# Golbstein/Keras-segmentation-deeplab-v3.1

Hardware: AMD Instinct MI355X
Metric: images/sec fwd+bwd, 512x512 MobileNetV2 OS=16, 21 classes (higher is better)
Workload: dtype f32; 1 GPU; Deeplabv3(backbone='mobilenetv2', input_shape=(512,512,3), classes=21, OS=16) head=deeplab: fwd + sparse-xent loss + bwd + Adam, BN batch mode, dropout 0.1; global_batch=128, per_gpu_batch=128, parallelism=dp1, hipgraph=True, matrix_math=f32, dist_strict=False, backward_fork=False

## Files before the change

keras-segmentation-deeplab-v3.1_amd/csrc/pwws.hip:

```cpp
#include "common.h"
#include "pwargs.h"
namespace {
using pw::GemmArgs;

template <int KQ, int TN, int OC>
__global__ __launch_bounds__(256, OC) void pw_fwd_ws_kernel(GemmArgs P) {
  constexpr int KH = 4 * KQ, K = 8 * KQ, NP = 32 * TN;
  __shared__ float Ws[K * NP];
  __shared__ float cf[2 * K];
  __shared__ float bs[NP];
  __shared__ float Cs[4 * 1024];
  static_assert(sizeof(float) * (K * NP + 2 * K + NP + 4 * 1024) * OC <= 160 * 1024, "weight-stationary kernel: OC workgroups do not fit a gfx950 CU's LDS");
  const int tid = threadIdx.x, lane = tid & 63;
  const int wave = __builtin_amdgcn_readfirstlane(tid >> 6);
  const int l31 = lane & 31, lhi = lane >> 5;
  const bool xform = (P.ka != nullptr);

  for (int i = tid; i < K * NP; i += 256) {
    const int k = i / NP, n = i % NP;
    Ws[i] = n < P.N ? P.b[(size_t)k * P.ldb + n] : 0.f;
  }
  for (int i = tid; i < K; i += 256) {
    cf[i] = xform ? P.ka[i] : 1.f;
    cf[K + i] = xform ? P.kc[i] : 0.f;
  }
  for (int i = tid; i < NP; i += 256) bs[i] = (P.bias && i < P.N) ? P.bias[i] : 0.f;
  float st1[TN], st2[TN];
#pragma unroll
  for (int j = 0; j < TN; j++) st1[j] = st2[j] = 0.f;
  __syncthreads();

  const int nfull = P.M >> 5;
  const int gw = blockIdx.x * 4 + wave, GW = gridDim.x * 4;
  float *const cw = Cs + wave * 1024;
  const float *const wfrag = Ws + KH * lhi * NP + l31;
  const float *const cfs = cf + KH * lhi, *const cft = cf + K + KH * lhi;
  const int c4 = (lane & 7) * 4, r0 = lane >> 3;
  const int c4l = c4 % (P.N - 32 * (TN - 1));

  f32x4 nx[KQ];
  auto load_tile = [&](int t) {
    const int row = min(t * 32 + l31, P.M - 1);
    const float *p = P.a + (size_t)row * P.lda + KH * lhi;
#pragma unroll
    for (int j = 0; j < KQ; j++) nx[j] = ld4(p + 4 * j);
  };
  auto mfma_tile = [&](f32x16 (&acc)[TN], int next) {
#pragma unroll
    for (int q = 0; q < KQ; q++) {
      const f32x4 v = dl3_act4(ld4(cfs + 4 * q) * nx[q] + ld4(cft + 4 * q), P.a_act);
#pragma unroll
      for (int e = 0; e < 4; e++)
#pragma unroll
        for (int j = 0; j < TN; j++)
          acc[j] = __builtin_amdgcn_mfma_f32_32x32x2f32(v[e], wfrag[(4 * q + e) * NP + j * 32], acc[j], 0, 0, 0);
    }
    __builtin_amdgcn_sched_barrier(0);
    if (next >= 0) load_tile(next);
    __builtin_amdgcn_sched_barrier(0);
  };

  if (gw < nfull) load_tile(gw);
  __builtin_amdgcn_s_waitcnt(0x0F70);
  for (int t = gw; t < nfull; t += GW) {
    f32x16 acc[TN];
#pragma unroll
    for (int j = 0; j < TN; j++)
#pragma unroll
      for (int r = 0; r < 16; r++) acc[j][r] = 0.f;
    mfma_tile(acc, t + GW < nfull ? t + GW : -1);
    float *const cp = P.c + (size_t)(t * 32 + r0) * P.ldc;
#pragma unroll
    for (int j = 0; j < TN; j++) {
      const float bj = bs[j * 32 + l31];
#pragma unroll
      for (int r = 0; r < 16; r++) {
        const float v = acc[j][r] + bj;
        st1[j] += v;
        st2[j] += v * v;
        cw[((r & 3) + 8 * (r >> 2) + 4 * lhi) * 32 + l31] = v;
      }
      __builtin_amdgcn_wave_barrier();
      const int cc = (j == TN - 1) ? c4l : c4;
      f32x4 o[4];
#pragma unroll
      for (int p = 0; p < 4; p++) o[p] = ld4(cw + (r0 + 8 * p) * 32 + cc);
#pragma unroll
      for (int p = 0; p < 4; p++) st4_nt(cp + (size_t)(8 * p) * P.ldc + j * 32 + cc, o[p]);
      __builtin_amdgcn_wave_barrier();
    }
  }
  if ((P.M & 31) != 0 && gw == nfull % GW) {
    f32x16 acc[TN];
#pragma unroll
    for (int j = 0; j < TN; j++)
#pragma unroll
      for (int r = 0; r < 16; r++) acc[j][r] = 0.f;
    load_tile(nfull);
    mfma_tile(acc, -1);
    const int m0 = nfull * 32;
#pragma unroll
    for (int j = 0; j < TN; j++) {
      const int col = j * 32 + l31;
      const float bj = bs[col];
#pragma unroll
      for (int r = 0; r < 16; r++) {
        const int row = m0 + (r & 3) + 8 * (r >> 2) + 4 * lhi;
        const float v = acc[j][r] + bj;
        if (row < P.M && col < P.N) {
          st1[j] += v;
          st2[j] += v * v;
          P.c[(size_t)row * P.ldc + col] = v;
        }
      }
    }
  }

  if (P.stat_mode != 0) {
    __syncthreads();
    float *sred = Cs;
#pragma unroll
    for (int j = 0; j < TN; j++) {
      const float a1 = st1[j] + __shfl_xor(st1[j], 32, 64), a2 = st2[j] + __shfl_xor(st2[j], 32, 64);
      if (lhi == 0) {
        sred[(wave * NP + j * 32 + l31) * 2 + 0] = a1;
        sred[(wave * NP + j * 32 + l31) * 2 + 1] = a2;
      }
    }
    __syncthreads();
    for (int cl = tid; cl < NP; cl += 256) {
      if (cl < P.N) {
        float a1 = 0.f, a2 = 0.f;
#pragma unroll
        for (int w = 0; w < 4; w++) {
          a1 += sred[(w * NP + cl) * 2 + 0];
          a2 += sred[(w * NP + cl) * 2 + 1];
        }
        P.part[((size_t)blockIdx.x * P.N + cl) * 2 + 0] = a1;
        P.part[((size_t)blockIdx.x * P.N + cl) * 2 + 1] = a2;
        for (int r = blockIdx.x + (int)gridDim.x; r < P.part_rows; r += (int)gridDim.x) {
          P.part[((size_t)r * P.N + cl) * 2 + 0] = 0.f;
          P.part[((size_t)r * P.N + cl) * 2 + 1] = 0.f;
        }
      }
    }
  }
}

#ifndef DL3_WS2_XPRE_TN
#define DL3_WS2_XPRE_TN 4
#endif
template <int KQ, int TN, int NW, bool BWD = false, bool TWO = false, bool ADD = false, bool FLAT = false>
__global__ __launch_bounds__(64 * NW) void pw_ws2_kernel(GemmArgs P) {
  static_assert(BWD || (!TWO && !ADD), "two-tensor operand / residual addend: bwd-data only");
  static_assert(!FLAT || (!BWD && TN == 1), "packed narrow output: forward, one column block");
  constexpr bool XPRE = BWD && !TWO && TN <= DL3_WS2_XPRE_TN;
  constexpr int KH = 4 * KQ, K = 8 * KQ, NP = 32 * TN;
  __shared__ __attribute__((aligned(16))) float Ws[K * NP];
  __shared__ __attribute__((aligned(16))) float cf[(TWO ? 3 : 2) * K];
  __shared__ __attribute__((aligned(16))) float bs[BWD ? 4 * NP : NP];
  __shared__ __attribute__((aligned(16))) float Cs[NW * 1024];
  static_assert(sizeof(float) * (K * NP + 3 * K + 4 * NP + NW * 1024) <= 160 * 1024, "gfx950: 160 KB of LDS per CU");
  const int tid = threadIdx.x, lane = tid & 63;
  const int wave = __builtin_amdgcn_readfirstlane(tid >> 6);
  const int l31 = lane & 31, lhi = lane >> 5;
  const int nwg = gridDim.x * gridDim.y, b = blockIdx.y * gridDim.x + blockIdx.x;
  const int xq = nwg >> 3, xr = nwg & 7, xcd = b & 7;
  const int lid = (xcd < xr ? xcd * (xq + 1) : xr * (xq + 1) + (xcd - xr) * xq) + (b >> 3);
  const int ct = lid % gridDim.x, rg = lid / gridDim.x, nrg = gridDim.y;
  const int n0 = ct * NP;
  const bool xform = (P.ka != nullptr);

  for (int i = tid; i < K * NP; i += 64 * NW) {
    const int k = i / NP, n = n0 + i % NP;
    Ws[i] = n < P.N ? P.b[(size_t)k * P.ldb + n] : 0.f;
  }
  for (int i = tid; i < K; i += 64 * NW) {
    cf[i] = xform ? P.ka[i] : 1.f;
    cf[K + i] = xform ? P.kc[i] : 0.f;
    if constexpr (TWO) cf[2 * K + i] = P.kb[i];
  }
  for (int i = tid; i < NP; i += 64 * NW) {
    const int col = min(n0 + i, P.N - 1);
    if constexpr (BWD) {
      bs[i] = P.ep_scale ? P.ep_scale[col] : 1.f;
      bs[NP + i] = P.ep_scale ? P.ep_shift[col] : 0.f;
      bs[2 * NP + i] = P.stat_mode == 2 ? P.ep_mean[col] : 0.f;
      bs[3 * NP + i] = P.stat_mode == 2 ? P.ep_invstd[col] : 0.f;
    } else {
      bs[i] = (P.bias && n0 + i < P.N) ? P.bias[n0 + i] : 0.f;
    }
  }
  float st1[TN], st2[TN];
#pragma unroll
  for (int j = 0; j < TN; j++) st1[j] = st2[j] = 0.f;
  f32x4 q1[BWD ? TN : 1], q2[BWD ? TN : 1];
  if constexpr (BWD) {
#pragma unroll
    for (int j = 0; j < TN; j++) q1[j] = q2[j] = splat4(0.f);
  }
  __syncthreads();

  const int nfull = P.M >> 5;
  const int gw = rg * NW + wave, GW = nrg * NW;
  float *const cw = Cs + wave * 1024;
  const float *const wfrag = Ws + KH * lhi * NP + l31;
  const float *const cfs = cf + KH * lhi, *const cft = cf + K + KH * lhi;
  const int c4 = (lane & 7) * 4, r0 = lane >> 3;
  const int ncol = min(NP, P.N - n0);
  const int jl = (ncol - 1) >> 5;
  const int c4l = FLAT ? 0 : c4 % (ncol - 32 * jl);

  constexpr int NCH = BWD ? KQ / 2 : 4;
  static_assert(NCH % 2 == 0, "an even number of chunks per tile");
  constexpr int SQ = KQ / NCH;
  static_assert(KQ % NCH == 0, "the reduction must split into an even number of equal chunks");
  f32x4 nx[2][SQ], ny[2][TWO ? SQ : 1];
  auto req = [&](int t, int c, int sl) __attribute__((always_inline)) {
    const int row = min(t * 32 + l31, P.M - 1);
    const float *p = P.a + (size_t)row * P.lda + KH * lhi + 4 * SQ * c;
#pragma unroll
    for (int j = 0; j < SQ; j++) nx[sl][j] = ld4(p + 4 * j);
    if constexpr (TWO) {
      const float *p2 = P.a2 + (size_t)row * P.lda2 + KH * lhi + 4 * SQ * c;
#pragma unroll
      for (int j = 0; j < SQ; j++) ny[sl][j] = ld4(p2 + 4 * j);
    }
  };
  auto mfma_tile = [&](f32x16 (&acc)[TN], int t, int tn) __attribute__((always_inline)) {
    float bf[2][TN];
#pragma unroll
    for (int j = 0; j < TN; j++) bf[0][j] = wfrag[j * 32];
#pragma unroll
    for (int c = 0; c < NCH; c++) {
#pragma unroll
      for (int q = 0; q < SQ; q++) {
        const int kq = SQ * c + q;
        f32x4 v;
        if constexpr (TWO) {
          v = ld4(cfs + 4 * kq) * nx[c & 1][q] + ld4(cft + 4 * kq);
          v += ld4(cf + 2 * K + KH * lhi + 4 * kq) * ny[c & 1][q];
        } else if constexpr (BWD) {
          v = nx[c & 1][q];
        } else {
          v = dl3_act4(ld4(cfs + 4 * kq) * nx[c & 1][q] + ld4(cft + 4 * kq), P.a_act);
        }
#pragma unroll
        for (int e = 0; e < 4; e++) {
          const int ks = 4 * kq + e, cur = ks & 1;
          if (ks + 1 < KH) {
#pragma unroll
            for (int j = 0; j < TN; j++) bf[cur ^ 1][j] = wfrag[(ks + 1) * NP + j * 32];
          }
#pragma unroll
          for (int j = 0; j < TN; j++) acc[j] = __builtin_amdgcn_mfma_f32_32x32x2f32(v[e], bf[cur][j], acc[j], 0, 0, 0);
          __builtin_amdgcn_sched_group_barrier(0x100, TN, 0);
          __builtin_amdgcn_sched_group_barrier(0x008, TN, 0);
        }
      }
      __builtin_amdgcn_sched_barrier(0);
      if (c + 2 < NCH) req(t, c + 2, c & 1);
      else req(tn, c + 2 - NCH, c & 1);
      __builtin_amdgcn_sched_barrier(0);
    }
  };

  if (gw < nfull) {
    req(gw, 0, 0);
    req(gw, 1, 1);
  }
  __builtin_amdgcn_s_waitcnt(0x0F70);
  for (int t = gw; t < nfull; t += GW) {
    f32x16 acc[TN];
#pragma unroll
    for (int j = 0; j < TN; j++)
#pragma unroll
      for (int r = 0; r < 16; r++) acc[j][r] = 0.f;
    f32x4 xq[BWD ? 2 : 1][BWD ? 4 : 1], aq[BWD ? 2 : 1][ADD ? 4 : 1];
    if constexpr (XPRE) {
      int le = lane, c4le = c4l;
      asm volatile("" : "+v"(le), "+v"(c4le));
      const int c4 = (le & 7) * 4, r0 = le >> 3, c4l = c4le;
      const float *const xp0 = P.ep_x + (size_t)(t * 32 + r0) * P.ld_epx + n0;
      const float *const ap0 = ADD ? P.ep_add + (size_t)(t * 32 + r0) * P.ld_add + n0 : nullptr;
#pragma unroll
      for (int jj = 0; jj < (TN < 2 ? TN : 2); jj++) {
        const int cc_ = jj < jl ? jj * 32 + c4 : jl * 32 + c4l;
#pragma unroll
        for (int p = 0; p < 4; p++) {
          xq[jj][p] = ld4(xp0 + (size_t)(8 * p) * P.ld_epx + cc_);
          if constexpr (ADD) aq[jj][p] = ld4(ap0 + (size_t)(8 * p) * P.ld_add + cc_);
        }
      }
    }
    mfma_tile(acc, t, t + GW < nfull ? t + GW : t);
    if constexpr (BWD) {
      int le = lane, c4le = c4l;
      asm volatile("" : "+v"(le), "+v"(c4le));
      const int c4 = (le & 7) * 4, r0 = le >> 3, l31 = le & 31, lhi = le >> 5, c4l = c4le;
      float *const cp = P.c + (size_t)(t * 32 + r0) * P.ldc + n0;
      const float *const xp = P.ep_x + (size_t)(t * 32 + r0) * P.ld_epx + n0;
      const float *const ap = ADD ? P.ep_add + (size_t)(t * 32 + r0) * P.ld_add + n0 : nullptr;
      if constexpr (!XPRE) {
#pragma unroll
        for (int p = 0; p < 4; p++) {
          xq[0][p] = ld4(xp + (size_t)(8 * p) * P.ld_epx + (0 == jl ? c4l : c4));
          if constexpr (ADD) aq[0][p] = ld4(ap + (size_t)(8 * p) * P.ld_add + (0 == jl ? c4l : c4));
        }
      }
#pragma unroll
      for (int j = 0; j < TN; j++) {
        if (j <= jl) {
          if (!XPRE && j + 1 <= jl) {
#pragma unroll
            for (int p = 0; p < 4; p++) {
              xq[(j + 1) & 1][p] = ld4(xp + (size_t)(8 * p) * P.ld_epx + (j + 1) * 32 + (j + 1 == jl ? c4l : c4));
              if constexpr (ADD) aq[(j + 1) & 1][p] = ld4(ap + (size_t)(8 * p) * P.ld_add + (j + 1) * 32 + (j + 1 == jl ? c4l : c4));
            }
          }
#pragma unroll
          for (int r = 0; r < 16; r++) cw[((r & 3) + 8 * (r >> 2) + 4 * lhi) * 32 + l31] = acc[j][r];
          __builtin_amdgcn_wave_barrier();
          const int cc = (j == jl) ? c4l : c4;
          const f32x4 es = ld4(bs + j * 32 + cc), et = ld4(bs + NP + j * 32 + cc);
          const f32x4 mu = ld4(bs + 2 * NP + j * 32 + cc), is = ld4(bs + 3 * NP + j * 32 + cc);
          const float own = (cc == c4) ? 1.f : 0.f;
#pragma unroll
          for (int p = 0; p < 4; p++) {
            const f32x4 x = xq[j & 1][p];
            f32x4 o = ld4(cw + (r0 + 8 * p) * 32 + cc) * dl3_mask4(es * x + et, P.ep_act);
            if constexpr (ADD) o += P.add_scale * aq[j & 1][p];
            st4_nt(cp + (size_t)(8 * p) * P.ldc + j * 32 + cc, o);
            q1[j] += own * o;
            q2[j] += own * (o * ((x - mu) * is));
          }
          if (XPRE && j + 2 <= jl) {
            __builtin_amdgcn_sched_barrier(0);
#pragma unroll
            for (int p = 0; p < 4; p++) {
              xq[j & 1][p] = ld4(xp + (size_t)(8 * p) * P.ld_epx + (j + 2) * 32 + (j + 2 == jl ? c4l : c4));
              if constexpr (ADD) aq[j & 1][p] = ld4(ap + (size_t)(8 * p) * P.ld_add + (j + 2) * 32 + (j + 2 == jl ? c4l : c4));
            }
          }
          __builtin_amdgcn_wave_barrier();
        }
      }
    } else if constexpr (FLAT) {
      const float bj = bs[l31];
      float *const cq = cw + 4 * lhi * P.N + l31;
#pragma unroll
      for (int r = 0; r < 16; r++) {
        const float v = acc[0][r] + bj;
        st1[0] += v;
        st2[0] += v * v;
        if (l31 < P.N) cq[((r & 3) + 8 * (r >> 2)) * P.N] = v;
      }
      __builtin_amdgcn_wave_barrier();
      float *const cp = P.c + (size_t)t * 32 * P.N;
#pragma unroll
      for (int p = 0; p < 4; p++) {
        const int piece = lane + 64 * p;
        if (piece < 8 * P.N) st4_nt(cp + 4 * piece, ld4(cw + 4 * piece));
      }
      __builtin_amdgcn_wave_barrier();
    } else {
    float *const cp = P.c + (size_t)(t * 32 + r0) * P.ldc + n0;
#pragma unroll
    for (int j = 0; j < TN; j++) {
      if (j <= jl) {
        const float bj = bs[j * 32 + l31];
#pragma unroll
        for (int r = 0; r < 16; r++) {
          const float v = acc[j][r] + bj;
          st1[j] += v;
          st2[j] += v * v;
          cw[((r & 3) + 8 * (r >> 2) + 4 * lhi) * 32 + l31] = v;
        }
        __builtin_amdgcn_wave_barrier();
        const int cc = (j == jl) ? c4l : c4;
        f32x4 o[4];
#pragma unroll
        for (int p = 0; p < 4; p++) o[p] = ld4(cw + (r0 + 8 * p) * 32 + cc);
#pragma unroll
        for (int p = 0; p < 4; p++) st4_nt(cp + (size_t)(8 * p) * P.ldc + j * 32 + cc, o[p]);
        __builtin_amdgcn_wave_barrier();
      }
    }
    }
  }
  if ((P.M & 31) != 0 && gw == nfull % GW) {
    f32x16 acc[TN];
#pragma unroll
    for (int j = 0; j < TN; j++)
#pragma unroll
      for (int r = 0; r < 16; r++) acc[j][r] = 0.f;
    __builtin_amdgcn_s_waitcnt(0x0F70);
    req(nfull, 0, 0);
    req(nfull, 1, 1);
    mfma_tile(acc, nfull, nfull);
    const int m0 = nfull * 32;
#pragma unroll
    for (int j = 0; j < TN; j++) {
      const int col = n0 + j * 32 + l31;
      const float bj = BWD ? 0.f : bs[j * 32 + l31];
#pragma unroll
      for (int r = 0; r < 16; r++) {
        const int row = m0 + (r & 3) + 8 * (r >> 2) + 4 * lhi;
        float v = acc[j][r] + bj;
        if (row < P.M && col < P.N) {
          if constexpr (BWD) {
            const float x = P.ep_x[(size_t)row * P.ld_epx + col];
            v *= dl3_act_mask(bs[j * 32 + l31] * x + bs[NP + j * 32 + l31], P.ep_act);
            if constexpr (ADD) v += P.add_scale * P.ep_add[(size_t)row * P.ld_add + col];
            st1[j] += v;
            st2[j] += v * ((x - bs[2 * NP + j * 32 + l31]) * bs[3 * NP + j * 32 + l31]);
          } else {
            st1[j] += v;
            st2[j] += v * v;
          }
          P.c[(size_t)row * P.ldc + col] = v;
        }
      }
    }
  }

  if (P.stat_mode != 0) {
    __syncthreads();
    float *sred = Cs;
    if constexpr (BWD) {
#pragma unroll
      for (int j = 0; j < TN; j++) {
#pragma unroll
        for (int o = 8; o <= 32; o <<= 1) {
#pragma unroll
          for (int e = 0; e < 4; e++) {
            q1[j][e] += __shfl_xor(q1[j][e], o, 64);
            q2[j][e] += __shfl_xor(q2[j][e], o, 64);
          }
        }
        if (lane < 8) {
#pragma unroll
          for (int e = 0; e < 4; e++) {
            sred[(wave * NP + j * 32 + c4 + e) * 2 + 0] = q1[j][e];
            sred[(wave * NP + j * 32 + c4 + e) * 2 + 1] = q2[j][e];
          }
        }
      }
      __builtin_amdgcn_wave_barrier();
    }
#pragma unroll
    for (int j = 0; j < TN; j++) {
      const float a1 = st1[j] + __shfl_xor(st1[j], 32, 64), a2 = st2[j] + __shfl_xor(st2[j], 32, 64);
      if (lhi == 0) {
        sred[(wave * NP + j * 32 + l31) * 2 + 0] = (BWD ? sred[(wave * NP + j * 32 + l31) * 2 + 0] : 0.f) + a1;
        sred[(wave * NP + j * 32 + l31) * 2 + 1] = (BWD ? sred[(wave * NP + j * 32 + l31) * 2 + 1] : 0.f) + a2;
      }
    }
    __syncthreads();
    for (int cl = tid; cl < NP; cl += 64 * NW) {
      const int col = n0 + cl;
      if (col < P.N) {
        float a1 = 0.f, a2 = 0.f;
#pragma unroll
        for (int w = 0; w < NW; w++) {
          a1 += sred[(w * NP + cl) * 2 + 0];
          a2 += sred[(w * NP + cl) * 2 + 1];
        }
        P.part[((size_t)rg * P.N + col) * 2 + 0] = a1;
        P.part[((size_t)rg * P.N + col) * 2 + 1] = a2;
        for (int r = rg + nrg; r < P.part_rows; r += nrg) {
          P.part[((size_t)r * P.N + col) * 2 + 0] = 0.f;
          P.part[((size_t)r * P.N + col) * 2 + 1] = 0.f;
        }
      }
    }
  }
}

template <int TN, int NW>
__global__ __launch_bounds__(64 * NW) void pw_narrowk_kernel(GemmArgs P) {
  constexpr int NP = 32 * TN;
  __shared__ __attribute__((aligned(16))) float Bs[32 * NP];
  __shared__ __attribute__((aligned(16))) float As[NW * 1024];
  __shared__ __attribute__((aligned(16))) float Cs[NW * 1024];
  static_assert(sizeof(float) * (32 * NP + 2 * NW * 1024) <= 160 * 1024, "gfx950: 160 KB of LDS per CU");
  const int tid = threadIdx.x, lane = tid & 63;
  const int wave = __builtin_amdgcn_readfirstlane(tid >> 6);
  const int l31 = lane & 31, lhi = lane >> 5;
  const int n0 = blockIdx.y * NP;
  for (int i = tid; i < 32 * NP; i += 64 * NW) {
    const int k = i / NP, n = n0 + i % NP;
    Bs[i] = (k < P.K && n < P.N) ? P.b[(size_t)k * P.ldb + n] : 0.f;
  }
  __syncthreads();
  const int KS = (P.K + 1) >> 1;
  const int npc = 8 * P.K;
  const int nfull = P.M >> 5;
  const int gw = blockIdx.x * NW + wave, GW = gridDim.x * NW;
  float *const as = As + wave * 1024, *const cw = Cs + wave * 1024;
  const int c4 = (lane & 7) * 4, r0 = lane >> 3;
  f32x4 f[4];
  auto req = [&](int t) __attribute__((always_inline)) {
    const float *p = P.a + (size_t)t * 32 * P.K;
#pragma unroll
    for (int q = 0; q < 4; q++)
      if (lane + 64 * q < npc) f[q] = ld4(p + 4 * (lane + 64 * q));
  };
  auto products = [&](f32x16 (&acc)[TN]) __attribute__((always_inline)) {
#pragma unroll
    for (int j = 0; j < TN; j++)
#pragma unroll
      for (int r = 0; r < 16; r++) acc[j][r] = 0.f;
    const float *ap = as + l31 * P.K + lhi * KS;
    const float *bp = Bs + lhi * KS * NP + l31;
    for (int s = 0; s < KS; s++) {
      const float a = (lhi * KS + s < P.K) ? ap[s] : 0.f;
#pragma unroll
      for (int j = 0; j < TN; j++) acc[j] = __builtin_amdgcn_mfma_f32_32x32x2f32(a, bp[s * NP + j * 32], acc[j], 0, 0, 0);
    }
  };
  if (gw < nfull) req(gw);
  for (int t = gw; t < nfull; t += GW) {
#pragma unroll
    for (int q = 0; q < 4; q++)
      if (lane + 64 * q < npc) st4(as + 4 * (lane + 64 * q), f[q]);
    __builtin_amdgcn_wave_barrier();
    req(t + GW < nfull ? t + GW : t);
    f32x16 acc[TN];
    products(acc);
    float *const cp = P.c + (size_t)(t * 32 + r0) * P.ldc + n0 + c4;
#pragma unroll
    for (int j = 0; j < TN; j++) {
      if (n0 + j * 32 < P.N) {
#pragma unroll
        for (int r = 0; r < 16; r++) cw[((r & 3) + 8 * (r >> 2) + 4 * lhi) * 32 + l31] = acc[j][r];
        __builtin_amdgcn_wave_barrier();
        f32x4 o[4];
#pragma unroll
        for (int p = 0; p < 4; p++) o[p] = ld4(cw + (r0 + 8 * p) * 32 + c4);
#pragma unroll
        for (int p = 0; p < 4; p++) st4_nt(cp + (size_t)(8 * p) * P.ldc + j * 32, o[p]);
        __builtin_amdgcn_wave_barrier();
      }
    }
  }
  if ((P.M & 31) != 0 && gw == nfull % GW) {
    const int m0 = nfull * 32;
    const size_t total = (size_t)P.M * P.K;
    for (int i = lane; i < 32 * P.K; i += 64) {
      const size_t e = (size_t)m0 * P.K + i;
      as[i] = e < total ? P.a[e] : 0.f;
    }
    __builtin_amdgcn_wave_barrier();
    f32x16 acc[TN];
    products(acc);
#pragma unroll
    for (int j = 0; j < TN; j++) {
      const int col = n0 + j * 32 + l31;
#pragma unroll
      for (int r = 0; r < 16; r++) {
        const int row = m0 + (r & 3) + 8 * (r >> 2) + 4 * lhi;
        if (row < P.M && col < P.N) P.c[(size_t)row * P.ldc + col] = acc[j][r];
      }
    }
  }
}
}

void pw::launch_ws(const GemmArgs &A, const GemmPlan &P, void *stream) {
  constexpr int NW = DL3_WS2_NW;
  const dim3 grid(P.grid[0], P.grid[1], P.grid[2]), blk(256), blkw(64 * NW);
#define DL3_GO(KERNEL_, BLK_) hipLaunchKernelGGL((KERNEL_), grid, BLK_, P.lds, (hipStream_t)stream, A)
  switch (P.kernel) {
    case PW_NARROW_FLAT: DL3_GO((pw_ws2_kernel<32, 1, NW, false, false, false, true>), blkw); break;
    case PW_NARROWK: DL3_GO((pw_narrowk_kernel<8, NW>), blkw); break;
    case PW_WS2:
      if (P.two) {
        if (P.add) DL3_GO((pw_ws2_kernel<48, 2, NW, true, true, true>), blkw);
        else DL3_GO((pw_ws2_kernel<48, 2, NW, true, true, false>), blkw);
      } else if (!P.fwd) {
        switch (P.tn) {
          case 5: DL3_GO((pw_ws2_kernel<20, 5, NW, true>), blkw); break;
          case 3: DL3_GO((pw_ws2_kernel<12, 3, NW, true>), blkw); break;
          default: DL3_GO((pw_ws2_kernel<8, 4, NW, true>), blkw); break;
        }
      } else {
        switch (P.tn) {
          case 5: DL3_GO((pw_ws2_kernel<20, 5, NW>), blkw); break;
          case 3: DL3_GO((pw_ws2_kernel<12, 3, NW>), blkw); break;
          default: DL3_GO((pw_ws2_kernel<8, 4, NW>), blkw); break;
        }
      }
      break;
    default:
      switch (P.kq * 10 + P.tn) {
        case 23: DL3_GO((pw_fwd_ws_kernel<2, 3, 4>), blk); break;
        case 35: DL3_GO((pw_fwd_ws_kernel<3, 5, 3>), blk); break;
        case 41: DL3_GO((pw_fwd_ws_kernel<4, 1, 4>), blk); break;
        case 46: DL3_GO((pw_fwd_ws_kernel<4, 6, 3>), blk); break;
        case 121: DL3_GO((pw_fwd_ws_kernel<12, 1, 4>), blk); break;
        case 181: DL3_GO((pw_fwd_ws_kernel<18, 1, 3>), blk); break;
        default: DL3_GO((pw_fwd_ws_kernel<24, 1, 3>), blk); break;
      }
  }
#undef DL3_GO
}
```

Measured before the change: 1345 img/s.

## Load A tiles as coalesced row lines and transpose through LDS in ws2 GEMM

Adds an alternative A-operand path in the weight-stationary pointwise GEMM. Each wave loads contiguous 16-float segments of 8 rows per instruction, applies the BN/activation transform, writes the result to a swizzled per-wave LDS scratch, and reads it back in MFMA fragment order. This replaces the per-lane strided row loads and is meant to improve global-memory coalescing for KQ==8 and two-tensor variants. The cost is extra LDS traffic and wave barriers on every chunk, plus more register use for the staging buffers.

```diff
diff --git a/keras-segmentation-deeplab-v3.1_amd/csrc/pwws.hip b/keras-segmentation-deeplab-v3.1_amd/csrc/pwws.hip
--- a/keras-segmentation-deeplab-v3.1_amd/csrc/pwws.hip
+++ b/keras-segmentation-deeplab-v3.1_amd/csrc/pwws.hip
@@ -149,6 +149,9 @@
 
 #ifndef DL3_WS2_XPRE_TN
 #define DL3_WS2_XPRE_TN 4
+#endif
+#ifndef DL3_WS2_LINES
+#define DL3_WS2_LINES 7
 #endif
 template <int KQ, int TN, int NW, bool BWD = false, bool TWO = false, bool ADD = false, bool FLAT = false>
 __global__ __launch_bounds__(64 * NW) void pw_ws2_kernel(GemmArgs P) {
@@ -211,6 +214,7 @@
   const int jl = (ncol - 1) >> 5;
   const int c4l = FLAT ? 0 : c4 % (ncol - 32 * jl);
 
+  constexpr bool LINES = (TWO && (DL3_WS2_LINES & 1)) || (KQ == 8 && BWD && !TWO && (DL3_WS2_LINES & 2)) || (KQ == 8 && !BWD && (DL3_WS2_LINES & 4));
   constexpr int NCH = BWD ? KQ / 2 : 4;
   static_assert(NCH % 2 == 0, "an even number of chunks per tile");
   constexpr int SQ = KQ / NCH;
@@ -227,7 +231,84 @@
       for (int j = 0; j < SQ; j++) ny[sl][j] = ld4(p2 + 4 * j);
     }
   };
+  constexpr int NCL = LINES ? KH / 16 : 2;
+  static_assert(!LINES || KH % 32 == 0, "line chunks: whole pairs per tile");
+  f32x4 lx[2][4], ly[TWO ? 2 : 1][4];
+  const int lr = lane >> 3, ls = lane & 7;
+  const int lk = KH * (ls >> 2) + 4 * (ls & 3);
+  auto req_pair = [&](int t, int c) __attribute__((always_inline)) {
+#pragma unroll
+    for (int p = 0; p < 4; p++) {
+      const int row = min(t * 32 + 8 * p + lr, P.M - 1);
+      const float *q = P.a + (size_t)row * P.lda + lk + 16 * c;
+      const float *q2 = TWO ? P.a2 + (size_t)row * P.lda2 + lk + 16 * c : nullptr;
+#pragma unroll
+      for (int h = 0; h < 2; h++) {
+        lx[h][p] = ld4(q + 16 * h);
+        if constexpr (TWO) ly[h][p] = ld4(q2 + 16 * h);
+      }
+    }
+  };
+  auto mfma_tile_lines = [&](f32x16 (&acc)[TN], int t, int tn) __attribute__((always_inline)) {
+    float bf[2][TN];
+#pragma unroll
+    for (int j = 0; j < TN; j++) bf[0][j] = wfrag[j * 32];
+    float *const wq = cw + lr * 32 + 4 * (ls ^ (lr >> 1));
+    const float *const rq = cw + l31 * 32;
+    const int rs = (l31 >> 1) & 7;
+    const float *const cfw = cf + lk;
+#pragma unroll
+    for (int c = 0; c < NCL; c++) {
+      const int sl = c & 1;
+      f32x4 ca, cc, cb;
+      if constexpr (TWO || !BWD) {
+        ca = ld4(cfw + 16 * c);
+        cc = ld4(cfw + K + 16 * c);
+      }
+      if constexpr (TWO) cb = ld4(cfw + 2 * K + 16 * c);
+#pragma unroll
+      for (int p = 0; p < 4; p++) {
+        f32x4 v;
+        if constexpr (TWO) {
+          v = ca * lx[sl][p] + cc;
+          v += cb * ly[sl][p];
+        } else if constexpr (BWD) {
+          v = lx[sl][p];
+        } else {
+          v = dl3_act4(ca * lx[sl][p] + cc, P.a_act);
+        }
+        st4(wq + p * 256 + ((p & 1) ? ((ls & 4) ? -16 : 16) : 0), v);
+      }
+      __builtin_amdgcn_wave_barrier();
+      if (c & 1) {
+        __builtin_amdgcn_sched_barrier(0);
+        if (c + 1 < NCL) req_pair(t, c + 1);
+        else req_pair(tn, 0);
+        __builtin_amdgcn_sched_barrier(0);
+      }
+      f32x4 va[4];
+#pragma unroll
+      for (int i = 0; i < 4; i++) va[i] = ld4(rq + 4 * ((4 * lhi + i) ^ rs));
+      __builtin_amdgcn_wave_barrier();
+#pragma unroll
+      for (int i = 0; i < 4; i++) {
+#pragma unroll
+        for (int e = 0; e < 4; e++) {
+          const int ks = 16 * c + 4 * i + e, cur = ks & 1;
+          if (ks + 1 < KH) {
+#pragma unroll
+            for (int j = 0; j < TN; j++) bf[cur ^ 1][j] = wfrag[(ks + 1) * NP + j * 32];
+          }
+#pragma unroll
+          for (int j = 0; j < TN; j++) acc[j] = __builtin_amdgcn_mfma_f32_32x32x2f32(va[i][e], bf[cur][j], acc[j], 0, 0, 0);
+          __builtin_amdgcn_sched_group_barrier(0x100, TN, 0);
+          __builtin_amdgcn_sched_group_barrier(0x008, TN, 0);
+        }
+      }
+    }
+  };
   auto mfma_tile = [&](f32x16 (&acc)[TN], int t, int tn) __attribute__((always_inline)) {
+    if constexpr (LINES) return mfma_tile_lines(acc, t, tn);
     float bf[2][TN];
 #pragma unroll
     for (int j = 0; j < TN; j++) bf[0][j] = wfrag[j * 32];
@@ -266,8 +347,12 @@
   };
 
   if (gw < nfull) {
-    req(gw, 0, 0);
-    req(gw, 1, 1);
+    if constexpr (LINES) {
+      req_pair(gw, 0);
+    } else {
+      req(gw, 0, 0);
+      req(gw, 1, 1);
+    }
   }
   __builtin_amdgcn_s_waitcnt(0x0F70);
   for (int t = gw; t < nfull; t += GW) {
@@ -395,8 +480,12 @@
 #pragma unroll
       for (int r = 0; r < 16; r++) acc[j][r] = 0.f;
     __builtin_amdgcn_s_waitcnt(0x0F70);
-    req(nfull, 0, 0);
-    req(nfull, 1, 1);
+    if constexpr (LINES) {
+      req_pair(nfull, 0);
+    } else {
+      req(nfull, 0, 0);
+      req(nfull, 1, 1);
+    }
     mfma_tile(acc, nfull, nfull);
     const int m0 = nfull * 32;
 #pragma unroll
```

New measurement: 1350 img/s (median of 6 runs). No clear change (+0.4%).
